# tiems90/mosaic

Measured on AMD Instinct MI355X. Metric: PIP-join points/sec (H3 res 9) at 1/2/4/8 GPUs + achieved HBM GB/s, higher is better.
Workload: dtype f64

## Files before the change

### mosaic_amd/csrc/capi.cpp

```cpp
#include <hip/hip_runtime.h>

#include <algorithm>
#include <cmath>
#include <cstdarg>
#include <cstdio>
#include <cstring>
#include <cstdlib>
#include <string>
#include <memory>
#include <functional>
#include <mutex>
#include <vector>

#include "../../include/mosaic_arrow.h"
#include "../../include/mosaic_gpu.h"
#include "error.h"
#include "h3_core.h"
#include "kernels.h"
#include "parallel.h"
#include "poly_slots.h"
#include "capi_internal.h"
#include "chip_build.h"
#include "geom_decode.h"
#include "h3_glibc.h"
// ... 244 lines not shown
    if (v < 1 || v > mgpu::bin_max()) return bad();
    o.bin_count = v;
  } else if (k == "bin_min_mb") {
    if (v < 0) return bad();
    o.bin_min_mb = v;
  } else if (k == "bin_min_points") {
    if (v < 0) return bad();
    o.bin_min_points = v;
  } else if (k == "bin_xcd") {
    if (v != 0 && v != 1) return bad();
    o.bin_xcd = v;
  } else if (k == "bin_keys") {
    if (v != 0 && v != 1) return bad();
    o.bin_keys = v;
  } else if (k == "ring_batch") {
    if (v < 1) return bad();
    o.ring_batch = v;
  } else if (k == "bng_split") {
    if (v != 0 && v != 1) return bad();
    o.bng_split = v;
  } else if (k == "cfy_fine") {
    if (v != 0 && v != 1) return bad();
    o.cfy_fine = v;
  } else if (k == "count_lds_slots") {
    if (v < 0 || v > mgpu::kCountLdsSlotsMax) return bad();
    o.count_lds_slots = v;
  } else if (k == "count_groups") {
    if (v < 0 || v > mgpu::kCountGroupsMax) return bad();
    o.count_groups = v;
  } else if (k == "cellagg_groups") {
    if (v < 0 || v > mgpu::kCountGroupsMax) return bad();
    o.cellagg_groups = v;
  } else if (k == "cellagg_bin_min") {
    if (v < 0) return bad();
    o.cellagg_bin_min = v;
  } else if (k == "cellagg_lds") {
    if (v != 0 && v != 1) return bad();
    o.cellagg_lds = v;
  } else if (k == "kring_batch") {
    if (v < 0 || v > 2147483647LL) return bad();
    o.kring_batch = v;
  } else if (k == "polyfill_slab") {
    if (v < 256 || v > ((int64_t)1 << 28)) return bad();
    o.polyfill_slab = v;
  } else if (k == "geomring_slab") {
    if (v < 1 || v > ((int64_t)1 << 24)) return bad();
// ... 6 lines not shown
    o.spin_us = v;
  } else if (k == "raster" || k == "raster_bng") {
    if (v != 0 && v != 1) return bad();
    (k == "raster" ? o.raster : o.raster_bng) = v;
  } else if (k == "raster_sub") {
    if (!(v == 0 || (v >= 2 && v <= 16))) return bad();
    o.raster_sub = v;
  } else if (k == "raster_milli") {
    if (v < 10 || v > 1000) return bad();
    o.raster_milli = v;
  } else {
    return fail(MGPU_E_INVALID_ARG, "unknown option %s", key);
  }
  return MGPU_OK;
}

int32_t mgpu_ctx_get_option(const mgpu_ctx* ctx, const char* key, int64_t* v) {
  if (!ctx || !key || !v) return fail(MGPU_E_INVALID_ARG, "NULL argument");
  const mgpu_options& o = ctx->opt;
  const std::pair<const char*, int64_t> all[] = {
      {"h3_libm", o.h3_libm},       {"pipeline", o.pipeline}, {"bin_count", o.bin_count},
      {"bin_min_mb", o.bin_min_mb}, {"bin_min_points", o.bin_min_points}, {"bin_xcd", o.bin_xcd},
      {"bin_keys", o.bin_keys},     {"spin_us", o.spin_us},   {"ring_batch", o.ring_batch},       {"raster", o.raster},     {"raster_bng", o.raster_bng},
      {"bng_split", o.bng_split},   {"cfy_fine", o.cfy_fine}, {"count_lds_slots", o.count_lds_slots}, {"count_groups", o.count_groups},
      {"kring_batch", o.kring_batch}, {"cellagg_groups", o.cellagg_groups}, {"cellagg_lds", o.cellagg_lds}, {"cellagg_bin_min", o.cellagg_bin_min},
      {"raster_sub", o.raster_sub}, {"raster_milli", o.raster_milli}, {"polyfill_slab", o.polyfill_slab},
      {"geomring_slab", o.geomring_slab}, {"geomring_lds_slots", o.geomring_lds_slots}};
  for (const auto& kv : all)
    if (strcmp(kv.first, key) == 0) {
      *v = kv.second;
      return MGPU_OK;
    }
  return fail(MGPU_E_INVALID_ARG, "unknown option %s", key);
}

int32_t mgpu_ctx_reserve(mgpu_ctx* ctx, int64_t max_points) {
  if (!ctx) return fail(MGPU_E_INVALID_ARG, "ctx is NULL");
  if (int32_t st = set_device(ctx->device)) return st;
  const int64_t tiles = mgpu::join_tiles(max_points);
  return ensure_ws(ctx, tiles, max_points);
}

}

int32_t cells_impl(mgpu_ctx* ctx, int32_t is, int32_t res, const double* x, const double* y, int64_t n,
                          int64_t* out_cell, hipStream_t s, const uint8_t* valid, int64_t voff, mgpu_stats* stats) {
  auto* counters = (unsigned long long*)ctx->ws;
// ... 620 lines not shown
    j.x = ba.bx;
    j.y = ba.by;
    j.mixed_idx = nullptr;
    j.chunk_mixed = nullptr;
    j.poly_answers = 1;
    j.pos_of = ba.perm;
    j.mixed_res = (uint64_t*)(bb + o_res);
    j.group_sum = (uint32_t*)(bb + o_gperm);
    j.group_cand = (uint32_t*)(bb + o_gcand);
    ba.s.j = j;
    ba.s.chunk_pairs = (uint32_t*)(bb + o_pairs);
    ba.s.chunk_off = (uint64_t*)(bb + o_off);
    ba.s.point_id = point_id;
    ba.s.id_base = id_base;
    ba.s.capacity = capacity;
    ba.s.out_point = out_point;
    ba.s.out_poly = out_poly;
    HIP_TRY(hipMemsetAsync(bb + o_gperm, 0, align_up(nc * 4, 256) + nc * 4, s));
  } else if (!split) {
    HIP_TRY(hipMemsetAsync(base + L.gsum, 0, 2 * ((size_t)tiles / 32 + 1) * 4, s));
  }
  if (timed) HIP_TRY(hipEventRecord(ctx->ev0, s));
  if (split)
    HIP_TRY(mgpu::launch_split(is, sa, s, timed ? ctx->ev2 : nullptr, timed ? ctx->ev3 : nullptr, emit));
  else if (binned)
    HIP_TRY(mgpu::launch_binned(is, ba, s, timed ? ctx->ev3 : nullptr, timed ? ctx->ev2 : nullptr, emit));
  else
    HIP_TRY(mgpu::launch_join(is, a, e, s, timed ? ctx->ev2 : nullptr, emit));
  if (timed) HIP_TRY(hipEventRecord(ctx->ev1, s));
  auto& L2 = ctx->last;
  L2.split = split;
  L2.sargs = sa;
  L2.binned = binned;
  L2.bargs = ba;
  L2.chips = chips;
  L2.is = is;
  L2.res = res;
  L2.x = x;
  L2.y = y;
  L2.point_id = point_id;
  L2.id_base = id_base;
  L2.n = n;
  L2.pts_valid = valid;
  L2.pts_valid_off = valid_off;
  L2.emit = e;
  L2.jargs = a;
  L2.n_tiles = tiles;
// ... 745 lines not shown
```

### mosaic_amd/csrc/capi_internal.h

```cpp
#pragma once
#include <hip/hip_runtime.h>
#include <stdint.h>

#include "../../include/mosaic_gpu.h"
#include "chip_table.h"
#include "kernels.h"

struct mgpu_options {
  int64_t h3_libm = MGPU_LIBM_REFERENCE;
  int64_t pipeline = MGPU_PIPELINE_AUTO;
  int64_t bin_count = 64;
  int64_t bin_min_mb = 256;
  int64_t bin_min_points = 1 << 21;
  int64_t bin_xcd = 1;
  int64_t bin_keys = 0;
  int64_t spin_us = 2000;
  int64_t ring_batch = (int64_t)1 << 26;
  int64_t count_lds_slots = 4096;
  int64_t count_groups = 0;
  int64_t kring_batch = 0;
  int64_t cellagg_groups = 0;
  int64_t cellagg_lds = 1;
  int64_t cellagg_bin_min = (int64_t)1 << 22;
  int64_t polyfill_slab = (int64_t)1 << 24;
  int64_t geomring_slab = (int64_t)1 << 16;
  int64_t geomring_lds_slots = 0;
  int64_t bng_split = 0;
  int64_t cfy_fine = 1;
  int64_t raster = 1, raster_bng = 0, raster_sub = 16, raster_milli = 250;
};

struct mgpu_ctx {
  int device = 0;
  mgpu_options opt;
  void* ws = nullptr;
  size_t ws_bytes = 0;
  hipEvent_t ev0 = nullptr, ev1 = nullptr, ev2 = nullptr, ev3 = nullptr;
  void* comm = nullptr;
  void* split_ws = nullptr;
  size_t split_bytes = 0;
  void* bin_ws = nullptr;
  size_t bin_bytes = 0;
  uint64_t* tq = nullptr;
  int64_t tq_cap = 0;
  uint64_t* ovr = nullptr;
  int64_t ovr_cap = 0;
  uint64_t* pin = nullptr;
  uint64_t* pin_dev = nullptr;
  void* scratch = nullptr;
  size_t scratch_bytes = 0;
// ... 53 lines not shown
```

### mosaic_amd/csrc/kernels.h

```cpp
#pragma once
#include <hip/hip_runtime.h>
#include <stdint.h>

#include "../../include/mosaic_gpu.h"
#include "chip_table.h"

namespace mgpu {

struct JoinArgs {
  const double* x;
  const double* y;
  int64_t n;
  int64_t n_tiles;
  int res;
  int res_match;
  ChipTableView chips;
  uint32_t* tile_count;
  uint32_t* group_sum;
  uint32_t* group_cand;
  uint64_t* tile_where;
  uint64_t* recs;
  int64_t pool_cap;
  unsigned long long* pool_used;
  uint32_t* dirty;
// ... 26 lines not shown
  uint32_t* first;
};

struct SplitArgs {
  JoinArgs j;
  void* codes;
  uint32_t* chunk_pairs;
  uint32_t* chunk_mixed;
  uint16_t* mixed_idx;
  uint32_t* extra;
  uint64_t* chunk_off;
  const int64_t* point_id;
  int64_t id_base;
  int64_t capacity;
  int64_t* out_point;
  int32_t* out_poly;
  const uint32_t* redo_first = nullptr;
  const uint8_t* redo_affected = nullptr;
};
int64_t split_chunk();
int64_t split_chunk_tiles();
int64_t split_chunks(int64_t n);
hipError_t launch_split(int is, const SplitArgs& a, hipStream_t s, hipEvent_t after_classify, hipEvent_t after_mixed,
                        bool emit = true);
hipError_t launch_split_emit(int is, const SplitArgs& a, hipStream_t s);
bool fine_table_shape(const ChipTableView& t, uint32_t* sx, uint32_t* sy, uint32_t* bnx, uint32_t* bny);
hipError_t launch_fine_table(const ChipTableView& t, uint32_t sx, uint32_t sy, uint32_t bnx, uint32_t bny, uint8_t* out,
                             hipStream_t s);
hipError_t launch_split_redo(int is, const SplitArgs& sa, const RedoArgs& R, int64_t n, hipStream_t s,
                             bool emit = true);

struct BinArgs {
  SplitArgs s;
  const double* x;
  const double* y;
  double* bx;
  double* by;
  uint32_t* perm;
  uint64_t* res;
  uint32_t* cnt;
  uint32_t* pre;
  uint32_t* gsum;
  double x0, y0, inv_bx, inv_by;
  int32_t nbx, nby;
  int32_t xcd_runs;
  uint32_t* key;
};
// ... 107 lines not shown
```

### mosaic_amd/csrc/kernels.hip

```cpp
#include <hip/hip_runtime.h>
#include <stdint.h>
#include <type_traits>

#include <map>
#include <mutex>

#define H3T_QUAL static __constant__ const
#include "h3_core.h"
#include "bng_core.h"
#include "pip_core.h"
#include "h3_ring.h"
#include "kernels.h"
#include "raster.h"

namespace mgpu {

#ifndef MGPU_BLOCK
#define MGPU_BLOCK 64
#endif
constexpr int kBlock = MGPU_BLOCK;
constexpr int kItems = 4;
constexpr int kTile = kBlock * kItems;
constexpr int kStreamBlock = 256;
static_assert(kTile <= 1024, "point-in-tile indices are 10 bits");

constexpr uint64_t kNoDst = ~0ULL;
constexpr int kScanGroup = 32;

// ... 1090 lines not shown
    const uint32_t eI = (uint32_t)bng::d2i(px), nI = (uint32_t)bng::d2i(py), ed = t.bng_edge;
    const uint32_t col = div_fix(eI, ed, t.bng_inv_edge), row = div_fix(nI, ed, t.bng_inv_edge);
    const uint32_t u = div_fix(eI - col * ed, t.cell_ans_sw, t.cell_ans_inv_sw);
    const uint32_t v = div_fix(nI - row * ed, t.cell_ans_sw, t.cell_ans_inv_sw);
    const uint32_t ai = t.cell_ans_row[row - (uint32_t)t.dense[0].b0] + cell_ans_index(e);
    const uint16_t m = t.cell_ans[((size_t)ai * t.cell_ans_g + v) * t.cell_ans_g + u];
    if (m != kCellAnsMixed && m < 256u) return m;
  }
  return kPixMixed;
}

#ifndef MGPU_CFY_BLOCK
#define MGPU_CFY_BLOCK 512
#endif
constexpr int kCfyBlock = MGPU_CFY_BLOCK;
#ifndef MGPU_CFY_BATCH
#define MGPU_CFY_BATCH 4
#endif
#ifndef MGPU_CFY_WAVES
#define MGPU_CFY_WAVES 1
#endif
constexpr int kCfyBatch = MGPU_CFY_BATCH;

template <int N, bool FINE = false>
__device__ __forceinline__ void raster_class_batch(const ChipTableView& t, const uint16_t* blk, const uint32_t* band,
                                                   const uint32_t (&ri)[N], const uint32_t (&bi)[N],
                                                   const uint32_t (&sub)[N], uint32_t (&cl)[N]) {
  const uint32_t s2 = t.raster_sub_n * t.raster_sub_n;
  uint32_t c[N], bb[N], px[N], q[N];
  bool pix[N], ref[N];
#pragma unroll
  for (int k = 0; k < N; k++) {
    const uint32_t i = bi[k] != kNoPixel ? bi[k] : 0u;
    c[k] = FINE ? (uint32_t)((const uint8_t*)blk)[i] : (uint32_t)blk[i];
    bb[k] = band[sub[k] >> 16];
  }
#pragma unroll
  for (int k = 0; k < N; k++) {
    pix[k] = ri[k] < kRasterFull && (bi[k] == kNoPixel || c[k] == (FINE ? kFineLookup : (uint32_t)kPixMixed));
    px[k] = t.raster[pix[k] ? ri[k] : 0u];
  }
#pragma unroll
  for (int k = 0; k < N; k++) {
    ref[k] = pix[k] && px[k] >= 0x8000u && px[k] != kPixMixed;
    const uint64_t i = ((uint64_t)bb[k] + (px[k] & 0x7FFFu)) * s2 + (sub[k] & 0xFFFFu);
    q[k] = t.raster_sub[ref[k] ? i : 0ull];
  }
#pragma unroll
  for (int k = 0; k < N; k++)
    cl[k] = ri[k] >= kRasterFull ? (ri[k] == kRasterFull ? kPixMixed : kPixEmpty) : ref[k] ? q[k] : pix[k] ? px[k] : c[k];
}

__host__ __device__ __forceinline__ bool cfy_staged(const ChipTableView& t, uint32_t nblk) {
  return t.raster_blk && nblk && t.raster_band && t.raster_nband && !t.raster_pal && t.raster_sub && t.raster_sub_n &&
         t.raster_nx && t.raster_ny;
}

#ifndef MGPU_CFY_FINE_BLOCK
#define MGPU_CFY_FINE_BLOCK 768
#endif
constexpr int kCfyFineBlock = MGPU_CFY_FINE_BLOCK;
static_assert(kCfyFineBlock == 512 || kCfyFineBlock == 768, "the fine classify kernels' launch shapes");
constexpr size_t kCfyFineLds = kCfyFineBlock == 512 ? 53 * 1024 : 79 * 1024;
constexpr int kCfyFineWaves = kCfyFineBlock == 768 ? 6 : MGPU_CFY_WAVES;
__host__ __device__ __forceinline__ size_t cfy_fine_lds(uint32_t nfine, uint32_t nband) {
  return (((size_t)nfine + 3) & ~(size_t)3) + (size_t)nband * 4;
}

template <int IS, class F>
__device__ __forceinline__ void cfy_dispatch(bool staged, bool nulls, F& run) {
  if constexpr (IS == MGPU_H3) {
    if (staged) {
      if (nulls) run(std::true_type{}, std::true_type{});
      else run(std::true_type{}, std::false_type{});
    } else {
      if (nulls) run(std::false_type{}, std::true_type{});
      else run(std::false_type{}, std::false_type{});
    }
  } else {
    run(std::false_type{}, std::true_type{});
  }
}

template <int IS, int BLOCK = kCfyBlock, bool FINE = false>
__global__ __launch_bounds__(BLOCK) __attribute__((amdgpu_waves_per_eu(FINE ? kCfyFineWaves : MGPU_CFY_WAVES))) void classify_wave_kernel(SplitArgs sa, int64_t n_chunks) {
  using Code = typename CodeOf<IS>::T;
  static_assert(!FINE || IS == MGPU_H3, "raster_fine is a lonlat table");
  constexpr int kW = BLOCK / 64;
  constexpr int kItems = kChunk / 64;
// ... 28 lines not shown
      for (int k = 0; k < kCfyBatch; k++) {
        const int64_t p = c0 + (int64_t)(b + k) * 64 + lane;
        bx[k] = by[k] = 0.0;
        if (kFull || p < a.n) {
          bx[k] = __builtin_nontemporal_load(&a.x[p]);
          by[k] = __builtin_nontemporal_load(&a.y[p]);
        }
      }
      uint32_t ri[kCfyBatch], gix[kCfyBatch], sb[kCfyBatch], bi[kCfyBatch];
#pragma unroll
      for (int k = 0; k < kCfyBatch; k++) {
        ri[k] = kNoPixel;
        gix[k] = 0;
        sb[k] = 0;
        bi[k] = kNoPixel;
        const int64_t pk = c0 + (int64_t)(b + k) * 64 + lane;
        if ((kFull || pk < a.n) && (!kNulls || pt_valid(a.valid, a.valid_off, pk))) {
          bool ok = true;
          uint32_t g_ = 0, s_ = 0, b_ = kNoPixel;
          if (IS == MGPU_BNG && bng_grid) {
            const uint32_t m = bng_grid_class(a, pk, bx[k], by[k], &ok, &g_);
            ri[k] = m == kPixMixed ? kRasterFull : m;
          } else {
            ri[k] = raster_index<IS, FINE>(t, bx[k], by[k], &ok, &g_, &s_, &b_);
          }
          gix[k] = g_;
          sb[k] = s_;
          bi[k] = use_blk ? b_ : kNoPixel;
          any_bad |= !ok;
        }
      }
      uint32_t cl[kCfyBatch];
      uint64_t ge[kCfyBatch];
#ifndef MGPU_CFY_ABLATE
#define MGPU_CFY_ABLATE 0
#endif
      if constexpr (kStaged) {
        raster_class_batch<kCfyBatch, FINE>(t, s_blk, s_band, ri, bi, sb, cl);
#pragma unroll
        for (int k = 0; k < kCfyBatch; k++) ge[k] = 0ull;
      } else {
#pragma unroll
        for (int k = 0; k < kCfyBatch; k++) {
#if MGPU_CFY_ABLATE == 1
          cl[k] = ri[k] < kRasterFull ? (ri[k] & 1) : kPixEmpty;
#elif MGPU_CFY_ABLATE == 2
          cl[k] = ri[k] < kRasterFull && bi[k] != kNoPixel && s_blk[bi[k]] != kPixMixed ? s_blk[bi[k]] : kPixEmpty;
#elif MGPU_CFY_ABLATE == 3
          cl[k] = ri[k] < kRasterFull ? (bi[k] != kNoPixel && s_blk[bi[k]] != kPixMixed ? s_blk[bi[k]] : t.raster[ri[k]])
                                      : kPixEmpty;
#elif MGPU_CFY_ABLATE == 4
          cl[k] = ri[k] < kRasterFull ? t.raster[ri[k]] : kPixEmpty;
#elif MGPU_CFY_ABLATE == 5
          cl[k] = ri[k] < kRasterFull ? (bi[k] != kNoPixel && s_blk[bi[k]] != kPixMixed ? s_blk[bi[k]] : kPixMixed)
                                      : kPixEmpty;
#else
          if (IS == MGPU_BNG && bng_grid)
            cl[k] = ri[k] == kRasterFull ? kPixMixed : (ri[k] == kNoPixel ? kPixEmpty : ri[k]);
          else
            cl[k] = ri[k] < kRasterFull ? raster_class_blk(t, s_blk, ri[k], bi[k], sb[k], s_band)
                                        : (ri[k] == kRasterFull ? kPixMixed : kPixEmpty);
#endif
          if (IS == MGPU_BNG && bng_grid) ge[k] = gix[k];
          else ge[k] = (IS == MGPU_BNG && ri[k] < kRasterFull) ? t.grid[gix[k]] : 0ull;
        }
      }
#pragma unroll
      for (int k = 0; k < kCfyBatch; k++) {
        const int64_t p = c0 + (int64_t)(b + k) * 64 + lane;
        const bool valid = kFull || p < a.n;
        bool mixed = cl[k] == kPixMixed;
        Code code;
        if (IS == MGPU_H3) {
          code = (Code)cl[k];
          if (!mixed && cl[k] != kPixEmpty) {
            const uint32_t c = cl[k];
            pairs += c < t.raster_pc[0] ? 1u : c < t.raster_pc[1] ? 2u : c < t.raster_pc[2] ? 3u : c < t.raster_pc[3] ? 4u
                     : (uint32_t)__popc((uint32_t)(t.raster_cls[c] >> 32));
          }
        } else {
          const uint32_t first = (uint32_t)ge[k], m = cl[k];
          if (!mixed && m && !(m < 256u && first < (1u << 24))) mixed = true;
          code = (Code)(mixed ? kCodeMixed32 : (m ? (first << 8) | m : 0u));
          if (!mixed) pairs += __popc(m);
        }
        if (valid) MGPU_ST_INTER(code, &codes[p]);
        mixed = mixed && valid;
        const unsigned long long bal = __ballot(mixed);
        if (mixed) sa.mixed_idx[c0 + nmixed + (uint32_t)__popcll(bal & below)] = (uint16_t)((b + k) * 64 + lane);
        nmixed += (uint32_t)__popcll(bal);
      }
    }
    pairs = wave_sum_u32(pairs);
    if (lane == 0) {
      sa.chunk_pairs[ch] = pairs;
      sa.chunk_mixed[ch] = nmixed;
      a.group_cand[ch] = 0;
    }
  };
  auto run = [&](auto staged_c, auto nulls_c) {
    for (int64_t ch = (int64_t)blockIdx.x * kW + wave; ch < n_chunks; ch += ch_step) {
      if (IS == MGPU_H3 && (ch + 1) * kChunk <= a.n) {
        if constexpr (IS == MGPU_H3) run_chunk(ch, staged_c, nulls_c, std::true_type{});
      } else {
        run_chunk(ch, staged_c, nulls_c, std::false_type{});
      }
    }
  };
  if constexpr (FINE) {
    if (a.valid != nullptr) run(std::true_type{}, std::true_type{});
    else run(std::true_type{}, std::false_type{});
  } else {
    cfy_dispatch<IS>(cfy_staged(t, nblk), a.valid != nullptr, run);
  }
// ... 11 lines not shown
  static_assert(!FINE || IS == MGPU_H3, "raster_fine is a lonlat table");
  constexpr int kW = BLOCK / 64;
  constexpr int kPairItems = kChunk / 128;
  constexpr int kPB = kCfyBatch / 2 > 0 ? kCfyBatch / 2 : 1;
  constexpr int kPts = 2 * kPB;
  static_assert(kPairItems % kPB == 0, "MGPU_CFY_BATCH / 2 must divide the pair items per lane of a chunk");
  const JoinArgs& a = sa.j;
  const ChipTableView& t = a.chips;
  extern __shared__ uint16_t s_blk[];
  const int lane = threadIdx.x & 63, wave = threadIdx.x >> 6;
  const bool use_blk = IS == MGPU_H3 && (FINE || t.raster_blk != nullptr);
  const bool bng_grid = IS == MGPU_BNG && t.raster_mode == kRasterNone;
  const uint32_t nblk = use_blk ? (FINE ? t.fine_bnx * t.fine_bny : t.raster_bnx * t.raster_bny) : 0u;
  uint32_t* s_band = FINE ? (uint32_t*)s_blk + ((nblk + 3) >> 2) : (uint32_t*)(s_blk + ((nblk + 1) & ~1u));
  if (FINE) {
    for (uint32_t i = threadIdx.x; i < ((nblk + 3) >> 2); i += BLOCK) ((uint32_t*)s_blk)[i] = ((const uint32_t*)t.raster_fine)[i];
  } else if (use_blk) {
    for (uint32_t i = threadIdx.x; i < nblk; i += BLOCK) s_blk[i] = t.raster_blk[i];
  }
  if (IS == MGPU_H3)
    for (uint32_t i = threadIdx.x; i < t.raster_nband; i += BLOCK) s_band[i] = t.raster_band[i];
  __syncthreads();
  Code* codes = (Code*)sa.codes;
  const unsigned long long below = (1ull << lane) - 1ull;
  bool any_bad = false;
  const int64_t ch_step = (int64_t)gridDim.x * kW;
  auto run_chunk = [&](int64_t ch, auto staged_c, auto nulls_c, auto full_c) {
    constexpr bool kStaged = decltype(staged_c)::value, kNulls = decltype(nulls_c)::value, kFull = decltype(full_c)::value;
    const int64_t c0 = ch * kChunk;
    uint32_t pairs = 0, nmixed = 0;
    for (int b = 0; b < kPairItems; b += kPB) {
      double X[kPts], Y[kPts];
#pragma unroll
      for (int k = 0; k < kPB; k++) {
        const int64_t p = c0 + (int64_t)(b + k) * 128 + 2 * lane;
        if (kFull || p + 1 < a.n) {
          const dbl2_t vx = __builtin_nontemporal_load((const dbl2_t*)(a.x + p));
          const dbl2_t vy = __builtin_nontemporal_load((const dbl2_t*)(a.y + p));
          X[2 * k] = vx.x, X[2 * k + 1] = vx.y, Y[2 * k] = vy.x, Y[2 * k + 1] = vy.y;
        } else {
          X[2 * k] = Y[2 * k] = X[2 * k + 1] = Y[2 * k + 1] = 0.0;
          if (p < a.n) X[2 * k] = a.x[p], Y[2 * k] = a.y[p];
        }
      }
      uint32_t ri[kPts], gix[kPts], sb[kPts], bi[kPts];
#pragma unroll
      for (int j = 0; j < kPts; j++) {
        ri[j] = kNoPixel;
        gix[j] = 0;
        sb[j] = 0;
        bi[j] = kNoPixel;
        const int64_t pj = c0 + (int64_t)(b + j / 2) * 128 + 2 * lane + (j & 1);
        if ((kFull || pj < a.n) && (!kNulls || pt_valid(a.valid, a.valid_off, pj))) {
          bool ok = true;
          uint32_t g_ = 0, s_ = 0, b_ = kNoPixel;
          if (IS == MGPU_BNG && bng_grid) {
            const uint32_t m = bng_grid_class(a, pj, X[j], Y[j], &ok, &g_);
            ri[j] = m == kPixMixed ? kRasterFull : m;
          } else {
            ri[j] = raster_index<IS, FINE>(t, X[j], Y[j], &ok, &g_, &s_, &b_);
          }
          gix[j] = g_;
          sb[j] = s_;
          bi[j] = use_blk ? b_ : kNoPixel;
          any_bad |= !ok;
        }
      }
      uint32_t cl[kPts];
      uint64_t ge[kPts];
      if constexpr (kStaged) {
        raster_class_batch<kPts, FINE>(t, s_blk, s_band, ri, bi, sb, cl);
#pragma unroll
        for (int j = 0; j < kPts; j++) ge[j] = 0ull;
      } else {
#pragma unroll
        for (int j = 0; j < kPts; j++) {
          if (IS == MGPU_BNG && bng_grid) {
            cl[j] = ri[j] == kRasterFull ? kPixMixed : (ri[j] == kNoPixel ? kPixEmpty : ri[j]);
            ge[j] = gix[j];
          } else {
            cl[j] = ri[j] < kRasterFull ? raster_class_blk(t, s_blk, ri[j], bi[j], sb[j], s_band)
                                        : (ri[j] == kRasterFull ? kPixMixed : kPixEmpty);
            ge[j] = (IS == MGPU_BNG && ri[j] < kRasterFull) ? t.grid[gix[j]] : 0ull;
          }
        }
      }
      Code code[kPts];
      bool mixed[kPts];
#pragma unroll
      for (int j = 0; j < kPts; j++) {
        const int64_t pj = c0 + (int64_t)(b + j / 2) * 128 + 2 * lane + (j & 1);
        bool m = cl[j] == kPixMixed;
        if (IS == MGPU_H3) {
          code[j] = (Code)cl[j];
          if (!m && cl[j] != kPixEmpty) {
            const uint32_t c = cl[j];
            pairs += c < t.raster_pc[0] ? 1u : c < t.raster_pc[1] ? 2u : c < t.raster_pc[2] ? 3u : c < t.raster_pc[3] ? 4u
                     : (uint32_t)__popc((uint32_t)(t.raster_cls[c] >> 32));
          }
        } else {
          const uint32_t first = (uint32_t)ge[j], mm = cl[j];
          if (!m && mm && !(mm < 256u && first < (1u << 24))) m = true;
          code[j] = (Code)(m ? kCodeMixed32 : (mm ? (first << 8) | mm : 0u));
          if (!m) pairs += __popc(mm);
        }
        mixed[j] = m && (kFull || pj < a.n);
      }
#pragma unroll
      for (int k = 0; k < kPB; k++) {
        const int64_t p = c0 + (int64_t)(b + k) * 128 + 2 * lane;
        if (kFull || p + 1 < a.n) {
          if (sizeof(Code) == 2) {
            MGPU_ST_INTER((uint32_t)code[2 * k] | ((uint32_t)code[2 * k + 1] << 16), (uint32_t*)(codes + p));
          } else {
            typedef uint32_t u32x2_t __attribute__((ext_vector_type(2)));
            u32x2_t v;
            v.x = (uint32_t)code[2 * k];
            v.y = (uint32_t)code[2 * k + 1];
            MGPU_ST_INTER(v, (u32x2_t*)(codes + p));
          }
        } else if (p < a.n) {
          MGPU_ST_INTER(code[2 * k], &codes[p]);
        }
        const unsigned long long b0 = __ballot(mixed[2 * k]), b1 = __ballot(mixed[2 * k + 1]);
        const uint32_t r0 = nmixed + (uint32_t)__popcll(b0 & below) + (uint32_t)__popcll(b1 & below);
        const uint16_t li = (uint16_t)((b + k) * 128 + 2 * lane);
        if (mixed[2 * k]) sa.mixed_idx[c0 + r0] = li;
        if (mixed[2 * k + 1]) sa.mixed_idx[c0 + r0 + (mixed[2 * k] ? 1u : 0u)] = (uint16_t)(li + 1);
        nmixed += (uint32_t)(__popcll(b0) + __popcll(b1));
      }
    }
    pairs = wave_sum_u32(pairs);
    if (lane == 0) {
      sa.chunk_pairs[ch] = pairs;
      sa.chunk_mixed[ch] = nmixed;
      a.group_cand[ch] = 0;
    }
  };
  auto run = [&](auto staged_c, auto nulls_c) {
    for (int64_t ch = (int64_t)blockIdx.x * kW + wave; ch < n_chunks; ch += ch_step) {
      if (IS == MGPU_H3 && (ch + 1) * kChunk <= a.n) {
        if constexpr (IS == MGPU_H3) run_chunk(ch, staged_c, nulls_c, std::true_type{});
      } else {
        run_chunk(ch, staged_c, nulls_c, std::false_type{});
      }
    }
  };
  if constexpr (FINE) {
    if (a.valid != nullptr) run(std::true_type{}, std::true_type{});
    else run(std::true_type{}, std::false_type{});
  } else {
    cfy_dispatch<IS>(cfy_staged(t, nblk), a.valid != nullptr, run);
  }
  count_wave(&a.counters[2], any_bad);
}

#ifndef MGPU_MIXED_LEAN
#define MGPU_MIXED_LEAN 1
#endif
template <int IS>
__global__ __launch_bounds__(kBlock) MGPU_JOIN_ATTR void pip_mixed_kernel(JoinArgs a) {
  const uint32_t nm = a.chunk_mixed[blockIdx.x];
  if (threadIdx.x == 0 && nm > (uint32_t)kGTile) {
    const uint32_t more = (nm - 1) / kGTile;
    const uint32_t q = atomicAdd(a.n_extra, more);
// ... 1469 lines not shown
}

bool fine_table_shape(const ChipTableView& t, uint32_t* sx, uint32_t* sy, uint32_t* bnx, uint32_t* bny) {
  if (t.raster_mode != kRasterLonLat || !cfy_staged(t, t.raster_bnx * t.raster_bny)) return false;
  const uint32_t shapes[3][2] = {{2, 2}, {3, 2}, {2, 3}};
  for (const auto& sh : shapes) {
    const uint64_t nx = ((uint64_t)t.raster_nx + (1u << sh[0]) - 1) >> sh[0], ny = ((uint64_t)t.raster_ny + (1u << sh[1]) - 1) >> sh[1];
    if (nx * ny > kCfyFineLds || cfy_fine_lds((uint32_t)(nx * ny), t.raster_nband) > kCfyFineLds) continue;
    *sx = sh[0], *sy = sh[1], *bnx = (uint32_t)nx, *bny = (uint32_t)ny;
    return true;
  }
  return false;
}

hipError_t launch_fine_table(const ChipTableView& t, uint32_t sx, uint32_t sy, uint32_t bnx, uint32_t bny, uint8_t* out,
                             hipStream_t s) {
  const uint32_t nfine = bnx * bny;
  if (hipError_t e = hipMemsetAsync(out, (int)kFineLookup, ((size_t)nfine + 3) & ~(size_t)3, s)) return e;
  hipLaunchKernelGGL(fine_table_kernel, dim3((nfine + 255) / 256), dim3(256), 0, s, t.raster, t.raster_nx, t.raster_ny, sx,
                     sy, bnx, nfine, out);
  return hipGetLastError();
}

static void launch_classify_fine(const SplitArgs& a, int64_t nc, hipStream_t s) {
  const ChipTableView& ct = a.j.chips;
  const size_t lds = cfy_fine_lds(ct.fine_bnx * ct.fine_bny, ct.raster_nband);
  const int64_t wg = (nc + kCfyFineBlock / 64 - 1) / (kCfyFineBlock / 64);
  auto go = [&](auto kernel) {
    if (lds > 64 * 1024) hipFuncSetAttribute((const void*)kernel, hipFuncAttributeMaxDynamicSharedMemorySize, (int)lds);
    const int64_t grid = std::min<int64_t>(wg, (int64_t)resident_blocks((const void*)kernel, kCfyFineBlock, lds));
    hipLaunchKernelGGL(kernel, dim3((unsigned)grid), dim3(kCfyFineBlock), lds, s, a, nc);
  };
  if (MGPU_CFY_PAIR && ((((uintptr_t)a.j.x) | ((uintptr_t)a.j.y)) & 15) == 0)
    go(classify_pair_kernel<MGPU_H3, kCfyFineBlock, true>);
  else
    go(classify_wave_kernel<MGPU_H3, kCfyFineBlock, true>);
}

template <int IS>
static void launch_split_t(const SplitArgs& a, hipStream_t s, hipEvent_t after_classify, hipEvent_t after_mixed, bool emit) {
  const int64_t nc = split_chunks(a.j.n);
  const ChipTableView& ct = a.j.chips;
  const size_t nblk = (IS == MGPU_H3 && ct.raster_blk) ? (size_t)ct.raster_bnx * ct.raster_bny : 0;
  const size_t lds = IS == MGPU_H3 ? ((nblk + 1) & ~(size_t)1) * 2 + (size_t)ct.raster_nband * 4 : 0;
  const int64_t wg = (nc + kCfyBlock / 64 - 1) / (kCfyBlock / 64);
  const bool fine = IS == MGPU_H3 && ct.raster_fine;
  if (!fine && lds > 64 * 1024) {
    hipFuncSetAttribute((const void*)classify_pair_kernel<IS>, hipFuncAttributeMaxDynamicSharedMemorySize, (int)lds);
    hipFuncSetAttribute((const void*)classify_wave_kernel<IS>, hipFuncAttributeMaxDynamicSharedMemorySize, (int)lds);
  }
  if (fine) {
    launch_classify_fine(a, nc, s);
  } else if (MGPU_CFY_PAIR && ((((uintptr_t)a.j.x) | ((uintptr_t)a.j.y)) & 15) == 0) {
    const int64_t grid = std::min<int64_t>(wg, (int64_t)resident_blocks((const void*)classify_pair_kernel<IS>, kCfyBlock, lds));
    hipLaunchKernelGGL(classify_pair_kernel<IS>, dim3((unsigned)grid), dim3(kCfyBlock), lds, s, a, nc);
  } else {
    const int64_t grid = std::min<int64_t>(wg, (int64_t)resident_blocks((const void*)classify_wave_kernel<IS>, kCfyBlock, lds));
    hipLaunchKernelGGL(classify_wave_kernel<IS>, dim3((unsigned)grid), dim3(kCfyBlock), lds, s, a, nc);
  }
  if (after_classify) hipEventRecord(after_classify, s);
  hipLaunchKernelGGL(pip_mixed_kernel<IS>, dim3((unsigned)nc), dim3(kBlock), 0, s, a.j);
  const int64_t more = std::min<int64_t>(nc, (int64_t)resident_blocks((const void*)pip_mixed_more_kernel<IS>, kBlock, 0));
  hipLaunchKernelGGL(pip_mixed_more_kernel<IS>, dim3((unsigned)more), dim3(kBlock), 0, s, a.j);
  const int64_t fix = nc * kChunkTiles < kFixGrid ? nc * kChunkTiles : kFixGrid;
  hipLaunchKernelGGL((pip_mixed_fix_kernel<IS, 2>), dim3((unsigned)fix), dim3(kBlock), 0, s, a.j);
  if (after_mixed) hipEventRecord(after_mixed, s);
  hipLaunchKernelGGL(tile_scan_kernel, dim3(1), dim3(kScanBlock), 0, s, a.chunk_pairs, a.j.group_cand, nc,
                     a.chunk_off, a.j.counters);
  if (emit) launch_emit<IS>(a, nc, s);
}

hipError_t launch_split(int is, const SplitArgs& a, hipStream_t s, hipEvent_t after_classify, hipEvent_t after_mixed,
                        bool emit) {
  if (a.j.n <= 0) return hipSuccess;
  if (is == MGPU_H3)
    launch_split_t<MGPU_H3>(a, s, after_classify, after_mixed, emit);
  else
    launch_split_t<MGPU_BNG>(a, s, after_classify, after_mixed, emit);
  return hipGetLastError();
}

hipError_t launch_split_redo(int is, const SplitArgs& sa, const RedoArgs& R, int64_t n, hipStream_t s, bool emit) {
  if (n <= 0) return hipSuccess;
  const int64_t nc = split_chunks(sa.j.n);
  hipLaunchKernelGGL(chunk_unpair_kernel, dim3((unsigned)n), dim3(256), 0, s, sa.j, R);
  const int64_t most = n * kChunkTiles;
  const unsigned fix = (unsigned)(most < kFixGrid ? most : kFixGrid);
  if (is == MGPU_H3)
    hipLaunchKernelGGL((pip_mixed_fix_kernel<MGPU_H3, 2>), dim3(fix), dim3(kBlock), 0, s, sa.j);
  else
    hipLaunchKernelGGL((pip_mixed_fix_kernel<MGPU_BNG, 2>), dim3(fix), dim3(kBlock), 0, s, sa.j);
  hipLaunchKernelGGL(redo_compare_kernel, dim3((unsigned)((n + 255) / 256)), dim3(256), 0, s,
                     (const uint32_t*)sa.chunk_pairs, R, n);
  hipLaunchKernelGGL(tile_scan_kernel, dim3(1), dim3(kScanBlock), 0, s, sa.chunk_pairs, sa.j.group_cand, nc,
                     sa.chunk_off, sa.j.counters, (const uint32_t*)R.changed);
  SplitArgs sr = sa;
  sr.redo_first = R.first;
  sr.redo_affected = R.affected;
  if (!emit) return hipGetLastError();
  if (is == MGPU_H3)
    launch_emit<MGPU_H3>(sr, nc, s);
// ... 100 lines not shown
```

### mosaic_amd/csrc/raster.h

```cpp
#pragma once
#include <math.h>
#include <stdint.h>

#include "bng_core.h"
#include "chip_table.h"
#include "../../include/mosaic_gpu.h"

namespace mgpu {

constexpr uint32_t kNoPixel = 0xFFFFFFFFu;

MGPU_HDI bool pt_valid(const uint8_t* v, int64_t off, int64_t p) {
  if (!v) return true;
  const int64_t b = off + p;
  return (v[b >> 3] >> (b & 7)) & 1;
}

constexpr uint32_t kRasterFull = 0xFFFFFFFEu;
MGPU_HDI uint32_t div_fix(uint32_t v, uint32_t d, double inv) {
  const uint32_t q = (uint32_t)((double)v * inv);
  return q * d > v ? q - 1 : ((q + 1) * d <= v ? q + 1 : q);
}
template <int IS, bool FINE = false>
MGPU_HDI uint32_t raster_index(const ChipTableView& t, double px, double py, bool* ok, uint32_t* gi, uint32_t* sub,
// ... 21 lines not shown
  }
  *ok = isfinite(px) && isfinite(py);
  if (!*ok || !(px >= t.bbox[0] && px <= t.bbox[2] && py >= t.bbox[1] && py <= t.bbox[3])) return kNoPixel;
  const double tx = (px - t.raster_x0) * t.raster_inv_dx, ty = (py - t.raster_y0) * t.raster_inv_dy;
  uint32_t ix = (uint32_t)tx, iy = (uint32_t)ty;
  ix = ix < t.raster_nx ? ix : t.raster_nx - 1;
  iy = iy < t.raster_ny ? iy : t.raster_ny - 1;
  if (FINE) {
    if (blk) *blk = (iy >> t.fine_sy) * t.fine_bnx + (ix >> t.fine_sx);
  } else if (blk && t.raster_bshift) {
    *blk = (iy >> t.raster_bshift) * t.raster_bnx + (ix >> t.raster_bshift);
  }
  if (t.raster_sub_n) {
    const double S = (double)t.raster_sub_n;
    uint32_t u = (uint32_t)((tx - (double)ix) * S), v = (uint32_t)((ty - (double)iy) * S);
    u = u < t.raster_sub_n ? u : t.raster_sub_n - 1;
    v = v < t.raster_sub_n ? v : t.raster_sub_n - 1;
    *sub = v * t.raster_sub_n + u;
    if (t.raster_band) *sub |= (iy >> t.raster_band_shift) << 16;
  }
  return iy * t.raster_nx + ix;
}

#ifndef MGPU_RANK_SPEC
#define MGPU_RANK_SPEC 0
#endif
MGPU_HDI uint32_t raster_class(const ChipTableView& t, uint32_t ri, uint32_t sub, const uint32_t* band = nullptr) {
  if (t.raster_band) {
    uint32_t cl = t.raster[ri];
    if (cl >= 0x8000u && cl != kPixMixed) {
      const uint64_t b = (uint64_t)(band ? band : t.raster_band)[sub >> 16] + (cl & 0x7FFFu);
      const uint32_t i = sub & 0xFFFFu, s2 = t.raster_sub_n * t.raster_sub_n;
      if (t.raster_pal) {
        const uint64_t P = t.raster_pal[b];
        const uint32_t q = t.raster_idx2[b * (s2 >> 2) + (i >> 2)];
        const uint32_t c = (uint32_t)(P >> (16 * ((q >> (2 * (i & 3))) & 3))) & 0x7FFFu;
        cl = (P & kPalFull) ? t.raster_sub[(P & 0xFFFFFFFFull) * s2 + i] : (c == 0x7FFFu ? kPixMixed : c);
      } else {
        cl = t.raster_sub[b * s2 + i];
      }
    }
    return cl;
  }
#if MGPU_RANK_SPEC
  const RankWord w = t.raster_rank ? t.raster_rank[ri >> 5] : RankWord{0u, 0u};
  uint32_t cl = t.raster[ri];
// ... 23 lines not shown
```

Baseline: 119.0 billion.

## Add classify prefetch path, flat index/count variants, cached grid sizing and cfy_grid option

Adds a software-prefetch path to the fine classify kernel that issues the next batch's point loads while the raster lookups of the current batch are in flight. It also adds a branchless raster-index variant, a flat pair-count variant that defers popcount lookups, and mbcnt-based prefix counting. The prefetch and flat variants sit behind compile macros that default to off. Separately, occupancy queries and hipFuncSetAttribute calls are cached per kernel to cut host launch overhead, and a new cfy_grid option can cap the classify grid size.

```diff
diff --git a/mosaic_amd/csrc/capi.cpp b/mosaic_amd/csrc/capi.cpp
--- a/mosaic_amd/csrc/capi.cpp
+++ b/mosaic_amd/csrc/capi.cpp
@@ -290,6 +290,9 @@
   } else if (k == "cfy_fine") {
     if (v != 0 && v != 1) return bad();
     o.cfy_fine = v;
+  } else if (k == "cfy_grid") {
+    if (v < 0 || v > mgpu::kCountGroupsMax) return bad();
+    o.cfy_grid = v;
   } else if (k == "count_lds_slots") {
     if (v < 0 || v > mgpu::kCountLdsSlotsMax) return bad();
     o.count_lds_slots = v;
@@ -342,7 +345,7 @@
       {"h3_libm", o.h3_libm},       {"pipeline", o.pipeline}, {"bin_count", o.bin_count},
       {"bin_min_mb", o.bin_min_mb}, {"bin_min_points", o.bin_min_points}, {"bin_xcd", o.bin_xcd},
       {"bin_keys", o.bin_keys},     {"spin_us", o.spin_us},   {"ring_batch", o.ring_batch},       {"raster", o.raster},     {"raster_bng", o.raster_bng},
-      {"bng_split", o.bng_split},   {"cfy_fine", o.cfy_fine}, {"count_lds_slots", o.count_lds_slots}, {"count_groups", o.count_groups},
+      {"bng_split", o.bng_split},   {"cfy_fine", o.cfy_fine}, {"cfy_grid", o.cfy_grid},{"count_lds_slots", o.count_lds_slots}, {"count_groups", o.count_groups},
       {"kring_batch", o.kring_batch}, {"cellagg_groups", o.cellagg_groups}, {"cellagg_lds", o.cellagg_lds}, {"cellagg_bin_min", o.cellagg_bin_min},
       {"raster_sub", o.raster_sub}, {"raster_milli", o.raster_milli}, {"polyfill_slab", o.polyfill_slab},
       {"geomring_slab", o.geomring_slab}, {"geomring_lds_slots", o.geomring_lds_slots}};
@@ -1009,7 +1012,7 @@
   }
   if (timed) HIP_TRY(hipEventRecord(ctx->ev0, s));
   if (split)
-    HIP_TRY(mgpu::launch_split(is, sa, s, timed ? ctx->ev2 : nullptr, timed ? ctx->ev3 : nullptr, emit));
+    HIP_TRY(mgpu::launch_split(is, sa, s, timed ? ctx->ev2 : nullptr, timed ? ctx->ev3 : nullptr, emit, o.cfy_grid));
   else if (binned)
     HIP_TRY(mgpu::launch_binned(is, ba, s, timed ? ctx->ev3 : nullptr, timed ? ctx->ev2 : nullptr, emit));
   else
diff --git a/mosaic_amd/csrc/capi_internal.h b/mosaic_amd/csrc/capi_internal.h
--- a/mosaic_amd/csrc/capi_internal.h
+++ b/mosaic_amd/csrc/capi_internal.h
@@ -26,6 +26,7 @@
   int64_t geomring_slab = (int64_t)1 << 16;
   int64_t geomring_lds_slots = 0;
   int64_t bng_split = 0;
+  int64_t cfy_grid = 0;
   int64_t cfy_fine = 1;
   int64_t raster = 1, raster_bng = 0, raster_sub = 16, raster_milli = 250;
 };
diff --git a/mosaic_amd/csrc/kernels.h b/mosaic_amd/csrc/kernels.h
--- a/mosaic_amd/csrc/kernels.h
+++ b/mosaic_amd/csrc/kernels.h
@@ -72,7 +72,7 @@
 int64_t split_chunk_tiles();
 int64_t split_chunks(int64_t n);
 hipError_t launch_split(int is, const SplitArgs& a, hipStream_t s, hipEvent_t after_classify, hipEvent_t after_mixed,
-                        bool emit = true);
+                        bool emit = true, int64_t cfy_grid = 0);
 hipError_t launch_split_emit(int is, const SplitArgs& a, hipStream_t s);
 bool fine_table_shape(const ChipTableView& t, uint32_t* sx, uint32_t* sy, uint32_t* bnx, uint32_t* bny);
 hipError_t launch_fine_table(const ChipTableView& t, uint32_t sx, uint32_t sy, uint32_t bnx, uint32_t bny, uint8_t* out,
diff --git a/mosaic_amd/csrc/kernels.hip b/mosaic_amd/csrc/kernels.hip
--- a/mosaic_amd/csrc/kernels.hip
+++ b/mosaic_amd/csrc/kernels.hip
@@ -4,6 +4,7 @@
 
 #include <map>
 #include <mutex>
+#include <vector>
 
 #define H3T_QUAL static __constant__ const
 #include "h3_core.h"
@@ -1140,12 +1141,16 @@
 #endif
 constexpr int kCfyBatch = MGPU_CFY_BATCH;
 
-template <int N, bool FINE = false>
+struct CfyNothing {
+  __device__ __forceinline__ void operator()() const {}
+};
+template <int N, bool FINE = false, class U = CfyNothing>
 __device__ __forceinline__ void raster_class_batch(const ChipTableView& t, const uint16_t* blk, const uint32_t* band,
                                                    const uint32_t (&ri)[N], const uint32_t (&bi)[N],
-                                                   const uint32_t (&sub)[N], uint32_t (&cl)[N]) {
+                                                   const uint32_t (&sub)[N], uint32_t (&cl)[N], U under_pixels = U{}) {
   const uint32_t s2 = t.raster_sub_n * t.raster_sub_n;
   uint32_t c[N], bb[N], px[N], q[N];
+  uint16_t pw[N];
   bool pix[N], ref[N];
 #pragma unroll
   for (int k = 0; k < N; k++) {
@@ -1156,17 +1161,20 @@
 #pragma unroll
   for (int k = 0; k < N; k++) {
     pix[k] = ri[k] < kRasterFull && (bi[k] == kNoPixel || c[k] == (FINE ? kFineLookup : (uint32_t)kPixMixed));
-    px[k] = t.raster[pix[k] ? ri[k] : 0u];
-  }
+    pw[k] = t.raster[pix[k] ? ri[k] : 0u];
+    c[k] = ri[k] >= kRasterFull ? (ri[k] == kRasterFull ? kPixMixed : kPixEmpty) : c[k];
+  }
+  under_pixels();
 #pragma unroll
   for (int k = 0; k < N; k++) {
+    px[k] = pw[k];
     ref[k] = pix[k] && px[k] >= 0x8000u && px[k] != kPixMixed;
     const uint64_t i = ((uint64_t)bb[k] + (px[k] & 0x7FFFu)) * s2 + (sub[k] & 0xFFFFu);
     q[k] = t.raster_sub[ref[k] ? i : 0ull];
-  }
-#pragma unroll
-  for (int k = 0; k < N; k++)
-    cl[k] = ri[k] >= kRasterFull ? (ri[k] == kRasterFull ? kPixMixed : kPixEmpty) : ref[k] ? q[k] : pix[k] ? px[k] : c[k];
+    c[k] = pix[k] ? px[k] : c[k];
+  }
+#pragma unroll
+  for (int k = 0; k < N; k++) cl[k] = ref[k] ? q[k] : c[k];
 }
 
 __host__ __device__ __forceinline__ bool cfy_staged(const ChipTableView& t, uint32_t nblk) {
@@ -1183,6 +1191,48 @@
 constexpr int kCfyFineWaves = kCfyFineBlock == 768 ? 6 : MGPU_CFY_WAVES;
 __host__ __device__ __forceinline__ size_t cfy_fine_lds(uint32_t nfine, uint32_t nband) {
   return (((size_t)nfine + 3) & ~(size_t)3) + (size_t)nband * 4;
+}
+
+#ifndef MGPU_CFY_PREFETCH
+#define MGPU_CFY_PREFETCH 0
+#endif
+#ifndef MGPU_CFY_COUNT_FLAT
+#define MGPU_CFY_COUNT_FLAT 0
+#endif
+#ifndef MGPU_CFY_INDEX_FLAT
+#define MGPU_CFY_INDEX_FLAT 0
+#endif
+
+__device__ __forceinline__ uint32_t cfy_pairs(const ChipTableView& t, uint32_t c, bool live, uint32_t bit, uint32_t* many) {
+#if MGPU_CFY_COUNT_FLAT
+  const bool big = live && c >= t.raster_pc[3];
+  *many |= big ? bit : 0u;
+  const uint32_t k = 1u + (c >= t.raster_pc[0] ? 1u : 0u) + (c >= t.raster_pc[1] ? 1u : 0u) + (c >= t.raster_pc[2] ? 1u : 0u);
+  return live && !big ? k : 0u;
+#else
+  if (!live) return 0u;
+  return c < t.raster_pc[0] ? 1u : c < t.raster_pc[1] ? 2u : c < t.raster_pc[2] ? 3u : c < t.raster_pc[3] ? 4u
+         : (uint32_t)__popc((uint32_t)(t.raster_cls[c] >> 32));
+#endif
+}
+__device__ __forceinline__ uint32_t cfy_below(unsigned long long ballot, uint32_t acc) {
+  return __builtin_amdgcn_mbcnt_hi((uint32_t)(ballot >> 32), __builtin_amdgcn_mbcnt_lo((uint32_t)ballot, acc));
+}
+template <int IS, bool FINE>
+__device__ __forceinline__ uint32_t cfy_index(const ChipTableView& t, double x, double y, bool* ok, uint32_t* gi, uint32_t* sub,
+                                              uint32_t* blk) {
+  if constexpr (FINE && MGPU_CFY_INDEX_FLAT) return raster_index_flat(t, x, y, ok, sub, blk);
+  else return raster_index<IS, FINE>(t, x, y, ok, gi, sub, blk);
+}
+template <int N>
+__device__ __forceinline__ uint32_t cfy_pairs_many(const ChipTableView& t, const uint32_t (&cl)[N], uint32_t many) {
+  uint32_t pairs = 0;
+  if (MGPU_CFY_COUNT_FLAT && __any(many != 0u)) {
+#pragma unroll
+    for (int k = 0; k < N; k++)
+      if (many & (1u << k)) pairs += (uint32_t)__popc((uint32_t)(t.raster_cls[cl[k]] >> 32));
+  }
+  return pairs;
 }
 
 template <int IS, class F>
@@ -1257,7 +1307,7 @@
             const uint32_t m = bng_grid_class(a, pk, bx[k], by[k], &ok, &g_);
             ri[k] = m == kPixMixed ? kRasterFull : m;
           } else {
-            ri[k] = raster_index<IS, FINE>(t, bx[k], by[k], &ok, &g_, &s_, &b_);
+            ri[k] = cfy_index<IS, FINE>(t, bx[k], by[k], &ok, &g_, &s_, &b_);
           }
           gix[k] = g_;
           sb[k] = s_;
@@ -1300,6 +1350,7 @@
           else ge[k] = (IS == MGPU_BNG && ri[k] < kRasterFull) ? t.grid[gix[k]] : 0ull;
         }
       }
+      uint32_t many = 0;
 #pragma unroll
       for (int k = 0; k < kCfyBatch; k++) {
         const int64_t p = c0 + (int64_t)(b + k) * 64 + lane;
@@ -1308,11 +1359,7 @@
         Code code;
         if (IS == MGPU_H3) {
           code = (Code)cl[k];
-          if (!mixed && cl[k] != kPixEmpty) {
-            const uint32_t c = cl[k];
-            pairs += c < t.raster_pc[0] ? 1u : c < t.raster_pc[1] ? 2u : c < t.raster_pc[2] ? 3u : c < t.raster_pc[3] ? 4u
-                     : (uint32_t)__popc((uint32_t)(t.raster_cls[c] >> 32));
-          }
+          pairs += cfy_pairs(t, cl[k], !mixed && cl[k] != kPixEmpty, 1u << k, &many);
         } else {
           const uint32_t first = (uint32_t)ge[k], m = cl[k];
           if (!mixed && m && !(m < 256u && first < (1u << 24))) mixed = true;
@@ -1325,6 +1372,7 @@
         if (mixed) sa.mixed_idx[c0 + nmixed + (uint32_t)__popcll(bal & below)] = (uint16_t)((b + k) * 64 + lane);
         nmixed += (uint32_t)__popcll(bal);
       }
+      if (IS == MGPU_H3) pairs += cfy_pairs_many(t, cl, many);
     }
     pairs = wave_sum_u32(pairs);
     if (lane == 0) {
@@ -1382,7 +1430,6 @@
     for (uint32_t i = threadIdx.x; i < t.raster_nband; i += BLOCK) s_band[i] = t.raster_band[i];
   __syncthreads();
   Code* codes = (Code*)sa.codes;
-  const unsigned long long below = (1ull << lane) - 1ull;
   bool any_bad = false;
   const int64_t ch_step = (int64_t)gridDim.x * kW;
   auto run_chunk = [&](int64_t ch, auto staged_c, auto nulls_c, auto full_c) {
@@ -1418,7 +1465,7 @@
             const uint32_t m = bng_grid_class(a, pj, X[j], Y[j], &ok, &g_);
             ri[j] = m == kPixMixed ? kRasterFull : m;
           } else {
-            ri[j] = raster_index<IS, FINE>(t, X[j], Y[j], &ok, &g_, &s_, &b_);
+            ri[j] = cfy_index<IS, FINE>(t, X[j], Y[j], &ok, &g_, &s_, &b_);
           }
           gix[j] = g_;
           sb[j] = s_;
@@ -1447,17 +1494,14 @@
       }
       Code code[kPts];
       bool mixed[kPts];
+      uint32_t many = 0;
 #pragma unroll
       for (int j = 0; j < kPts; j++) {
         const int64_t pj = c0 + (int64_t)(b + j / 2) * 128 + 2 * lane + (j & 1);
         bool m = cl[j] == kPixMixed;
         if (IS == MGPU_H3) {
           code[j] = (Code)cl[j];
-          if (!m && cl[j] != kPixEmpty) {
-            const uint32_t c = cl[j];
-            pairs += c < t.raster_pc[0] ? 1u : c < t.raster_pc[1] ? 2u : c < t.raster_pc[2] ? 3u : c < t.raster_pc[3] ? 4u
-                     : (uint32_t)__popc((uint32_t)(t.raster_cls[c] >> 32));
-          }
+          pairs += cfy_pairs(t, cl[j], !m && cl[j] != kPixEmpty, 1u << j, &many);
         } else {
           const uint32_t first = (uint32_t)ge[j], mm = cl[j];
           if (!m && mm && !(mm < 256u && first < (1u << 24))) m = true;
@@ -1483,12 +1527,13 @@
           MGPU_ST_INTER(code[2 * k], &codes[p]);
         }
         const unsigned long long b0 = __ballot(mixed[2 * k]), b1 = __ballot(mixed[2 * k + 1]);
-        const uint32_t r0 = nmixed + (uint32_t)__popcll(b0 & below) + (uint32_t)__popcll(b1 & below);
+        const uint32_t r0 = cfy_below(b1, cfy_below(b0, nmixed));
         const uint16_t li = (uint16_t)((b + k) * 128 + 2 * lane);
         if (mixed[2 * k]) sa.mixed_idx[c0 + r0] = li;
         if (mixed[2 * k + 1]) sa.mixed_idx[c0 + r0 + (mixed[2 * k] ? 1u : 0u)] = (uint16_t)(li + 1);
         nmixed += (uint32_t)(__popcll(b0) + __popcll(b1));
       }
+      if (IS == MGPU_H3) pairs += cfy_pairs_many(t, cl, many);
     }
     pairs = wave_sum_u32(pairs);
     if (lane == 0) {
@@ -1497,10 +1542,99 @@
       a.group_cand[ch] = 0;
     }
   };
+  constexpr int kPF = MGPU_CFY_PREFETCH < kPB ? MGPU_CFY_PREFETCH : kPB;
+  auto load_items = [&](int64_t p0, auto k0_c, auto k1_c, dbl2_t (&PX)[kPB], dbl2_t (&PY)[kPB]) {
+#pragma unroll
+    for (int k = decltype(k0_c)::value; k < decltype(k1_c)::value; k++) {
+      const int64_t p = p0 + (int64_t)k * 128 + 2 * lane;
+      PX[k] = __builtin_nontemporal_load((const dbl2_t*)(a.x + p));
+      PY[k] = __builtin_nontemporal_load((const dbl2_t*)(a.y + p));
+    }
+  };
+  using I0 = std::integral_constant<int, 0>;
+  using IPF = std::integral_constant<int, kPF>;
+  using IPB = std::integral_constant<int, kPB>;
+  auto run_chunk_pf = [&](int64_t ch, auto nulls_c, dbl2_t (&PX)[kPB], dbl2_t (&PY)[kPB], bool next_full) {
+    constexpr bool kNulls = decltype(nulls_c)::value;
+    const int64_t c0 = ch * kChunk;
+    uint32_t pairs = 0, nmixed = 0;
+    auto batch = [&](int b, int64_t next_p0, auto prefetch_c) {
+      load_items(c0 + (int64_t)b * 128, IPF{}, IPB{}, PX, PY);
+      uint32_t ri[kPts], sb[kPts], bi[kPts];
+#pragma unroll
+      for (int j = 0; j < kPts; j++) {
+        ri[j] = kNoPixel;
+        sb[j] = 0;
+        bi[j] = kNoPixel;
+        const int64_t pj = c0 + (int64_t)(b + j / 2) * 128 + 2 * lane + (j & 1);
+        const double x = (j & 1) ? PX[j / 2].y : PX[j / 2].x, y = (j & 1) ? PY[j / 2].y : PY[j / 2].x;
+        const bool live = !kNulls || pt_valid(a.valid, a.valid_off, pj);
+        bool ok = true;
+        if constexpr (FINE && MGPU_CFY_INDEX_FLAT) {
+          ri[j] = raster_index_flat(t, x, y, &ok, &sb[j], &bi[j], live);
+          any_bad |= live && !ok;
+        } else if (live) {
+          uint32_t g_ = 0, s_ = 0, b_ = kNoPixel;
+          ri[j] = raster_index<IS, FINE>(t, x, y, &ok, &g_, &s_, &b_);
+          sb[j] = s_;
+          bi[j] = use_blk ? b_ : kNoPixel;
+          any_bad |= !ok;
+        }
+      }
+      uint32_t cl[kPts];
+      raster_class_batch<kPts, FINE>(t, s_blk, s_band, ri, bi, sb, cl, [&]() {
+        if constexpr (decltype(prefetch_c)::value) {
+          __builtin_amdgcn_sched_barrier(0);
+          load_items(next_p0, I0{}, IPF{}, PX, PY);
+          __builtin_amdgcn_sched_barrier(0);
+        }
+      });
+      Code code[kPts];
+      bool mixed[kPts];
+      uint32_t many = 0;
+#pragma unroll
+      for (int j = 0; j < kPts; j++) {
+        mixed[j] = cl[j] == kPixMixed;
+        code[j] = (Code)cl[j];
+        pairs += cfy_pairs(t, cl[j], !mixed[j] && cl[j] != kPixEmpty, 1u << j, &many);
+      }
+#pragma unroll
+      for (int k = 0; k < kPB; k++) {
+        const int64_t p = c0 + (int64_t)(b + k) * 128 + 2 * lane;
+        MGPU_ST_INTER((uint32_t)code[2 * k] | ((uint32_t)code[2 * k + 1] << 16), (uint32_t*)(codes + p));
+        const unsigned long long b0 = __ballot(mixed[2 * k]), b1 = __ballot(mixed[2 * k + 1]);
+        const uint32_t r0 = cfy_below(b1, cfy_below(b0, nmixed));
+        const uint16_t li = (uint16_t)((b + k) * 128 + 2 * lane);
+        if (mixed[2 * k]) sa.mixed_idx[c0 + r0] = li;
+        if (mixed[2 * k + 1]) sa.mixed_idx[c0 + r0 + (mixed[2 * k] ? 1u : 0u)] = (uint16_t)(li + 1);
+        nmixed += (uint32_t)(__popcll(b0) + __popcll(b1));
+      }
+      pairs += cfy_pairs_many(t, cl, many);
+    };
+    for (int b = 0; b < kPairItems; b += kPB) {
+      const bool last = b + kPB >= kPairItems;
+      if (!last || next_full)
+        batch(b, last ? (ch + ch_step) * kChunk : c0 + (int64_t)(b + kPB) * 128, std::true_type{});
+      else
+        batch(b, 0, std::false_type{});
+    }
+    pairs = wave_sum_u32(pairs);
+    if (lane == 0) {
+      sa.chunk_pairs[ch] = pairs;
+      sa.chunk_mixed[ch] = nmixed;
+      a.group_cand[ch] = 0;
+    }
+  };
   auto run = [&](auto staged_c, auto nulls_c) {
-    for (int64_t ch = (int64_t)blockIdx.x * kW + wave; ch < n_chunks; ch += ch_step) {
+    constexpr bool kPrefetch = MGPU_CFY_PREFETCH && FINE && sizeof(Code) == 2 && decltype(staged_c)::value;
+    const auto full = [&](int64_t ch) { return ch < n_chunks && (ch + 1) * kChunk <= a.n; };
+    int64_t ch = (int64_t)blockIdx.x * kW + wave;
+    dbl2_t PX[kPB] = {}, PY[kPB] = {};
+    if (kPrefetch && full(ch)) load_items(ch * kChunk, I0{}, IPF{}, PX, PY);
+    for (; ch < n_chunks; ch += ch_step) {
       if (IS == MGPU_H3 && (ch + 1) * kChunk <= a.n) {
-        if constexpr (IS == MGPU_H3) run_chunk(ch, staged_c, nulls_c, std::true_type{});
+        if constexpr (kPrefetch) run_chunk_pf(ch, nulls_c, PX, PY, full(ch + ch_step));
+        else if constexpr (IS == MGPU_H3) run_chunk(ch, staged_c, nulls_c, std::true_type{});
       } else {
         run_chunk(ch, staged_c, nulls_c, std::false_type{});
       }
@@ -3016,13 +3150,51 @@
   return hipGetLastError();
 }
 
-static void launch_classify_fine(const SplitArgs& a, int64_t nc, hipStream_t s) {
+static int classify_grid(const void* kernel, int block, size_t lds) {
+  struct Entry {
+    const void* kernel;
+    int block, dev;
+    size_t lds;
+    int grid;
+  };
+  struct Limit {
+    const void* kernel;
+    int dev;
+    size_t lds;
+  };
+  static std::mutex mu;
+  static std::vector<Entry> seen;
+  static std::vector<Limit> limits;
+  int dev = 0;
+  hipGetDevice(&dev);
+  std::lock_guard<std::mutex> lock(mu);
+  for (const Entry& e : seen)
+    if (e.kernel == kernel && e.block == block && e.dev == dev && e.lds == lds) return e.grid;
+  if (lds > 64 * 1024) {
+    Limit* l = nullptr;
+    for (Limit& q : limits)
+      if (q.kernel == kernel && q.dev == dev) l = &q;
+    if (!l) {
+      limits.push_back({kernel, dev, 0});
+      l = &limits.back();
+    }
+    if (lds > l->lds) {
+      hipFuncSetAttribute(kernel, hipFuncAttributeMaxDynamicSharedMemorySize, (int)lds);
+      l->lds = lds;
+    }
+  }
+  const int grid = resident_blocks(kernel, block, lds);
+  seen.push_back({kernel, block, dev, lds, grid});
+  return grid;
+}
+
+static void launch_classify_fine(const SplitArgs& a, int64_t nc, hipStream_t s, int64_t cfy_grid) {
   const ChipTableView& ct = a.j.chips;
   const size_t lds = cfy_fine_lds(ct.fine_bnx * ct.fine_bny, ct.raster_nband);
   const int64_t wg = (nc + kCfyFineBlock / 64 - 1) / (kCfyFineBlock / 64);
   auto go = [&](auto kernel) {
-    if (lds > 64 * 1024) hipFuncSetAttribute((const void*)kernel, hipFuncAttributeMaxDynamicSharedMemorySize, (int)lds);
-    const int64_t grid = std::min<int64_t>(wg, (int64_t)resident_blocks((const void*)kernel, kCfyFineBlock, lds));
+    int64_t grid = std::min<int64_t>(wg, (int64_t)classify_grid((const void*)kernel, kCfyFineBlock, lds));
+    if (cfy_grid > 0) grid = std::min(grid, cfy_grid);
     hipLaunchKernelGGL(kernel, dim3((unsigned)grid), dim3(kCfyFineBlock), lds, s, a, nc);
   };
   if (MGPU_CFY_PAIR && ((((uintptr_t)a.j.x) | ((uintptr_t)a.j.y)) & 15) == 0)
@@ -3032,25 +3204,26 @@
 }
 
 template <int IS>
-static void launch_split_t(const SplitArgs& a, hipStream_t s, hipEvent_t after_classify, hipEvent_t after_mixed, bool emit) {
+static void launch_split_t(const SplitArgs& a, hipStream_t s, hipEvent_t after_classify, hipEvent_t after_mixed, bool emit,
+                           int64_t cfy_grid) {
   const int64_t nc = split_chunks(a.j.n);
   const ChipTableView& ct = a.j.chips;
   const size_t nblk = (IS == MGPU_H3 && ct.raster_blk) ? (size_t)ct.raster_bnx * ct.raster_bny : 0;
   const size_t lds = IS == MGPU_H3 ? ((nblk + 1) & ~(size_t)1) * 2 + (size_t)ct.raster_nband * 4 : 0;
   const int64_t wg = (nc + kCfyBlock / 64 - 1) / (kCfyBlock / 64);
   const bool fine = IS == MGPU_H3 && ct.raster_fine;
-  if (!fine && lds > 64 * 1024) {
-    hipFuncSetAttribute((const void*)classify_pair_kernel<IS>, hipFuncAttributeMaxDynamicSharedMemorySize, (int)lds);
-    hipFuncSetAttribute((const void*)classify_wave_kernel<IS>, hipFuncAttributeMaxDynamicSharedMemorySize, (int)lds);
-  }
+  auto grid_of = [&](const void* kernel) {
+    const int64_t grid = std::min<int64_t>(wg, (int64_t)classify_grid(kernel, kCfyBlock, lds));
+    return cfy_grid > 0 ? std::min(grid, cfy_grid) : grid;
+  };
   if (fine) {
-    launch_classify_fine(a, nc, s);
+    launch_classify_fine(a, nc, s, cfy_grid);
   } else if (MGPU_CFY_PAIR && ((((uintptr_t)a.j.x) | ((uintptr_t)a.j.y)) & 15) == 0) {
-    const int64_t grid = std::min<int64_t>(wg, (int64_t)resident_blocks((const void*)classify_pair_kernel<IS>, kCfyBlock, lds));
-    hipLaunchKernelGGL(classify_pair_kernel<IS>, dim3((unsigned)grid), dim3(kCfyBlock), lds, s, a, nc);
+    hipLaunchKernelGGL(classify_pair_kernel<IS>, dim3((unsigned)grid_of((const void*)classify_pair_kernel<IS>)), dim3(kCfyBlock),
+                       lds, s, a, nc);
   } else {
-    const int64_t grid = std::min<int64_t>(wg, (int64_t)resident_blocks((const void*)classify_wave_kernel<IS>, kCfyBlock, lds));
-    hipLaunchKernelGGL(classify_wave_kernel<IS>, dim3((unsigned)grid), dim3(kCfyBlock), lds, s, a, nc);
+    hipLaunchKernelGGL(classify_wave_kernel<IS>, dim3((unsigned)grid_of((const void*)classify_wave_kernel<IS>)), dim3(kCfyBlock),
+                       lds, s, a, nc);
   }
   if (after_classify) hipEventRecord(after_classify, s);
   hipLaunchKernelGGL(pip_mixed_kernel<IS>, dim3((unsigned)nc), dim3(kBlock), 0, s, a.j);
@@ -3065,12 +3238,12 @@
 }
 
 hipError_t launch_split(int is, const SplitArgs& a, hipStream_t s, hipEvent_t after_classify, hipEvent_t after_mixed,
-                        bool emit) {
+                        bool emit, int64_t cfy_grid) {
   if (a.j.n <= 0) return hipSuccess;
   if (is == MGPU_H3)
-    launch_split_t<MGPU_H3>(a, s, after_classify, after_mixed, emit);
+    launch_split_t<MGPU_H3>(a, s, after_classify, after_mixed, emit, cfy_grid);
   else
-    launch_split_t<MGPU_BNG>(a, s, after_classify, after_mixed, emit);
+    launch_split_t<MGPU_BNG>(a, s, after_classify, after_mixed, emit, cfy_grid);
   return hipGetLastError();
 }
 
diff --git a/mosaic_amd/csrc/raster.h b/mosaic_amd/csrc/raster.h
--- a/mosaic_amd/csrc/raster.h
+++ b/mosaic_amd/csrc/raster.h
@@ -67,6 +67,29 @@
   return iy * t.raster_nx + ix;
 }
 
+MGPU_HDI uint32_t raster_index_flat(const ChipTableView& t, double px, double py, bool* ok, uint32_t* sub, uint32_t* blk,
+                                    bool live = true) {
+  *ok = isfinite(px) && isfinite(py);
+  const bool in = live && *ok && px >= t.bbox[0] && px <= t.bbox[2] && py >= t.bbox[1] && py <= t.bbox[3];
+  const double qx = in ? px : t.raster_x0, qy = in ? py : t.raster_y0;
+  const double tx = (qx - t.raster_x0) * t.raster_inv_dx, ty = (qy - t.raster_y0) * t.raster_inv_dy;
+  uint32_t ix = (uint32_t)tx, iy = (uint32_t)ty;
+  ix = ix < t.raster_nx ? ix : t.raster_nx - 1;
+  iy = iy < t.raster_ny ? iy : t.raster_ny - 1;
+  *blk = in ? (iy >> t.fine_sy) * t.fine_bnx + (ix >> t.fine_sx) : kNoPixel;
+  uint32_t s = 0;
+  if (t.raster_sub_n) {
+    const double S = (double)t.raster_sub_n;
+    uint32_t u = (uint32_t)((tx - (double)ix) * S), v = (uint32_t)((ty - (double)iy) * S);
+    u = u < t.raster_sub_n ? u : t.raster_sub_n - 1;
+    v = v < t.raster_sub_n ? v : t.raster_sub_n - 1;
+    s = v * t.raster_sub_n + u;
+    if (t.raster_band) s |= (iy >> t.raster_band_shift) << 16;
+  }
+  *sub = in ? s : 0u;
+  return in ? iy * t.raster_nx + ix : kNoPixel;
+}
+
 #ifndef MGPU_RANK_SPEC
 #define MGPU_RANK_SPEC 0
 #endif
```

Measured after the change: 119.0 billion, median of 2. Within noise of the previous version (+0.0%).
